# tlsfuzzer/tlslite-ng

Hardware: AMD Instinct MI355X
Metric: GiB/s device-resident record seal/open, AES-128-GCM + ChaCha20-Poly1305 16KiB (higher is better)
Workload: dtype u8

## Files before the change

tlslite-ng_amd/csrc/aes_bs.h:

```cpp
#pragma once
#include <stdint.h>
#if defined(__HIPCC__)
#include <hip/hip_runtime.h>
#endif

#if defined(__HIPCC__)
#define TG_BS_HD __host__ __device__ __forceinline__
#define TG_BS_MF __host__ __device__ __forceinline__
#else
#define TG_BS_HD static inline
#define TG_BS_MF inline
#endif

namespace tg {
namespace bs {

TG_BS_HD uint32_t bitmask(uint32_t w, int p) { return (uint32_t)((int32_t)(w << (31 - p)) >> 31); }

#if defined(__HIP_DEVICE_COMPILE__)
#define bop3(a, b, c, tt) __builtin_amdgcn_bitop3_b32((a), (b), (c), (tt))
#else
TG_BS_HD uint32_t bop3(uint32_t a, uint32_t b, uint32_t c, uint32_t tt) {
    uint32_t r = 0;
    for (int k = 0; k < 8; ++k)
        if ((tt >> k) & 1) r |= ((k & 4) ? a : ~a) & ((k & 2) ? b : ~b) & ((k & 1) ? c : ~c);
    return r;
}
#endif
TG_BS_HD uint32_t xor3(uint32_t a, uint32_t b, uint32_t c) { return bop3(a, b, c, 0x96); }

TG_BS_HD uint32_t perm(uint32_t hi, uint32_t lo, uint32_t sel) {
#if defined(__HIP_DEVICE_COMPILE__)
    return __builtin_amdgcn_perm(hi, lo, sel);
#else
    const uint64_t v = ((uint64_t)hi << 32) | lo;
    uint32_t r = 0;
    for (int i = 0; i < 4; ++i) r |= (uint32_t)((v >> (8 * ((sel >> (8 * i)) & 7))) & 0xff) << (8 * i);
    return r;
#endif
}

#include "aes_bs_sbox.h"

}
}
```

tlslite-ng_amd/csrc/aes_bs8.h:

```cpp
#pragma once
#include "aes_bs.h"
#include "keymath.h"

namespace tg {
namespace bs8 {

#if !defined(__HIP_DEVICE_COMPILE__)
using bs::bop3;
#endif
using bs::perm;
using bs::xor3;

TG_BS_HD uint32_t rotr_bytes(uint32_t x, int i) {
#if defined(__HIP_DEVICE_COMPILE__)
    return __builtin_amdgcn_alignbit(x, x, 8 * i);
#else
    return i ? (x >> (8 * i)) | (x << (32 - 8 * i)) : x;
#endif
}

TG_BS_HD uint32_t mask_word(const uint32_t* rk, int e) { return bs8_mask_word(rk, e); }

#if defined(__HIPCC__)
using Word4 = uint4;
// ... 206 lines not shown
            const uint32_t cw[4] = {c[b].x, c[b].y, c[b].z, c[b].w};
#pragma unroll
            for (int i = 0; i < 4; ++i) T[i] = xor3(a[i], a[(i + 1) & 3], cw[i]);
        }
#pragma unroll
        for (int i = 0; i < 4; ++i) {
            const uint32_t Tprev = b == 0 ? T7[i] : Tp[i];
            if (b == 1 || b == 3 || b == 4)
                s[i][b] = xor3(Tprev, T7[i], a[(i + 1) & 3]) ^ T[(i + 2) & 3];
            else
                s[i][b] = xor3(Tprev, a[(i + 1) & 3], T[(i + 2) & 3]);
        }
#pragma unroll
        for (int i = 0; i < 4; ++i) Tp[i] = T[i];
        TG_BS8_FENCE();
    }
}

struct TransposeMasks {
    uint32_t m4, m2, m1;
};
TG_BS_HD TransposeMasks transpose_masks() {
    TransposeMasks t{0x0f0f0f0fu, 0x33333333u, 0x55555555u};
#if defined(__HIP_DEVICE_COMPILE__)
    asm volatile("v_mov_b32 %0, 0x0f0f0f0f" : "=v"(t.m4));
    asm volatile("v_mov_b32 %0, 0x33333333" : "=v"(t.m2));
    asm volatile("v_mov_b32 %0, 0x55555555" : "=v"(t.m1));
#endif
    return t;
}

TG_BS_HD void transpose8(uint32_t* a, const TransposeMasks& tm) {
#pragma unroll
    for (int l = 2; l >= 0; --l) {
        const int m = 1 << l;
        const uint32_t mask = m == 4 ? tm.m4 : m == 2 ? tm.m2 : tm.m1;
#pragma unroll
        for (int r = 0; r < 8; ++r) {
            if (r & m) continue;
            const uint32_t x = a[r], y = a[r + m];
            uint32_t ys = y << m;
#if defined(__HIP_DEVICE_COMPILE__)
            if (m == 1) asm("v_add_u32 %0, %1, %1" : "=v"(ys) : "v"(y));
#endif
            a[r] = bop3(mask, x, ys, 0xca);
            a[r + m] = bop3(mask, x >> m, y, 0xca);
        }
    }
}

TG_BS_HD void to_blocks(uint32_t (*x)[8], uint32_t (*w)[8]) {
#pragma unroll
    for (int b = 0; b < 8; ++b) {
        const uint32_t s0 = x[0][b], s1 = x[1][b], s2 = x[2][b], s3 = x[3][b];
        const uint32_t A = perm(s1, s0, 0x07020500u);
        const uint32_t B = perm(s3, s2, 0x05000702u);
        const uint32_t A2 = perm(s1, s0, 0x04030601u);
        const uint32_t B2 = perm(s3, s2, 0x06010403u);
        w[0][b] = perm(B, A, 0x05040100u);
        w[2][b] = perm(B, A, 0x07060302u);
        w[1][b] = perm(B2, A2, 0x05040100u);
        w[3][b] = perm(B2, A2, 0x07060302u);
        TG_BS8_FENCE();
    }
    const TransposeMasks tm = transpose_masks();
#pragma unroll
    for (int q = 0; q < 4; ++q) {
        transpose8(w[q], tm);
        TG_BS8_FENCE();
    }
}

template <class KM, class = void>
struct RoundRows {
    static constexpr bool value = false;
};
template <class KM>
struct RoundRows<KM, decltype((void)KM::kRound)> {
    static constexpr bool value = KM::kRound;
};
template <class KM>
TG_BS_HD constexpr bool round_rows() { return RoundRows<KM>::value; }

template <int NR, class KM>
TG_BS_HD void encrypt(uint32_t (*s)[8], const KM& km, uint32_t (*w)[8], bool sub01 = true) {
    Word4 c[8];
    if constexpr (round_rows<KM>()) km.round(1, c);
    if (sub01) {
        bs::sbox(s[0]);
        TG_BS8_FENCE();
        bs::sbox(s[1]);
        TG_BS8_FENCE();
    }
    bs::sbox(s[2]);
    TG_BS8_FENCE();
    bs::sbox(s[3]);
    TG_BS8_FENCE();
    if constexpr (round_rows<KM>())
        mix_round_rows(s, c);
    else if constexpr (KM::kFolded)
        mix_round_folded(s, km, 1);
    else
        mix_round(s, km, 1);
#if defined(__HIP_DEVICE_COMPILE__)
#pragma unroll 1
#endif
    for (int r = 2; r < NR; ++r) {
        if constexpr (round_rows<KM>()) km.round(r, c);
#pragma unroll
        for (int i = 0; i < 4; ++i) {
            bs::sbox(s[i]);
            TG_BS8_FENCE();
        }
        if constexpr (round_rows<KM>())
            mix_round_rows(s, c);
        else if constexpr (KM::kFolded)
            mix_round_folded(s, km, r);
        else
            mix_round(s, km, r);
    }
#pragma unroll
    for (int i = 0; i < 4; ++i) {
        bs::sbox(s[i]);
        TG_BS8_FENCE();
    }
    to_blocks(s, w);
}

}
}
```

tlslite-ng_amd/csrc/aes_gcm_bs8.hip:

```cpp
#include <cstdlib>
#include <map>
#include <mutex>
#include <type_traits>
#include <utility>

#include "aes_bs8.h"
#include "aes_round.h"
#include "gcm_lane.h"
#include "ghash.h"
#include "options.h"
#include "runtime.h"

namespace tg {
namespace {

constexpr uint32_t kRecArea = 1536;

constexpr int kBs8Threads = 512;
constexpr int kBs8Recs = kBs8Threads / 8;
constexpr uint32_t kTeBase = 65536;
constexpr uint32_t kBs8Sbox = 65536;
constexpr uint32_t kBs8Jt = 65536 + 256;
constexpr uint32_t kBs8Keys = kBs8Jt + 256;
constexpr uint32_t kBs8RecBase = kBs8Keys + 2048;
constexpr size_t kBs8Lds = kBs8RecBase + (kBs8Threads / 64) * kRecArea;

extern __shared__ __attribute__((aligned(16))) uint4 g_lds_bs8[];

__device__ __forceinline__ uint32_t wave_max_u32(uint32_t v) {
#pragma unroll
    for (int off = 32; off >= 1; off >>= 1) {
        const uint32_t o = (uint32_t)__shfl_xor((int)v, off, 64);
        v = o > v ? o : v;
    }
    return __builtin_amdgcn_readfirstlane(v);
}

__device__ __forceinline__ uint32_t wave_min_u32(uint32_t v) {
#pragma unroll
    for (int off = 32; off >= 1; off >>= 1) {
        const uint32_t o = (uint32_t)__shfl_xor((int)v, off, 64);
        v = o < v ? o : v;
    }
    return __builtin_amdgcn_readfirstlane(v);
}

#if defined(TG_ROLE_PROBE)
__device__ unsigned long long g_rp[2][10];
struct RoleProbe {
    uint64_t last = 0;
    uint64_t acc[4] = {0, 0, 0, 0};
    __device__ __forceinline__ void start() { last = __builtin_amdgcn_s_memtime(); }
    __device__ __forceinline__ void mark(int k) {
        const uint64_t t = __builtin_amdgcn_s_memtime();
        acc[k] += t - last;
        last = t;
    }
    __device__ __forceinline__ void flush(bool trole, uint32_t blocks) {
        if ((threadIdx.x & 63u) == 0) {
            for (int k = 0; k < 4; ++k) atomicAdd(&g_rp[trole][k], (unsigned long long)acc[k]);
            atomicAdd(&g_rp[trole][5], 1ull);
            atomicAdd(&g_rp[trole][6], (unsigned long long)blocks);
        }
    }
};
__global__ void role_probe_print() {
    for (int r = 0; r < 2; ++r) {
        printf("ROLE_PROBE role %s setup %llu cipher %llu consume %llu tail %llu grab %llu jobs %llu blocks %llu span %llu waves %llu\n",
               r ? "ttable" : "bitsliced", g_rp[r][0], g_rp[r][1], g_rp[r][2], g_rp[r][3], g_rp[r][4], g_rp[r][5],
               g_rp[r][6], g_rp[r][7], g_rp[r][8]);
        for (int k = 0; k < 10; ++k) g_rp[r][k] = 0;
    }
}
#else
struct RoleProbe {
    __device__ __forceinline__ void start() {}
    __device__ __forceinline__ void mark(int) {}
    __device__ __forceinline__ void flush(bool, uint32_t) {}
};
#endif


template <int NR, int LPR = 8, class RK = RkLds>
__device__ __forceinline__ void t_half(uint32_t lane4, const RK& rk, const CtrCache& cc,
                                       uint32_t c0, bool win, const uint4& wc, uint32_t k0w, int h,
                                       uint4 (&ks)[4]) {
    uint32_t s[4][4];
#pragma unroll
    for (int q = 0; q < 4; ++q) {
        const uint32_t ctr = c0 + (uint32_t)LPR * (4 * h + q);
        if (win) {
            const uint32_t A = cc.k0 ^ rotl32(T2<3>((ctr << 24) ^ k0w, lane4), 8);
            s[q][0] = wc.x ^ T0<0>(A, lane4);
            s[q][1] = wc.y ^ rotl32(T2<3>(A, lane4), 8);
            s[q][2] = wc.z ^ T2<2>(A, lane4);
            s[q][3] = wc.w ^ rotl32(T0<1>(A, lane4), 8);
        } else {
            const uint32_t s3 = bswap32(ctr) ^ k0w;
            const uint32_t a0 = cc.k0 ^ rotl32(T2<3>(s3, lane4), 8);
            const uint32_t a1 = cc.k1 ^ T2<2>(s3, lane4);
            const uint32_t a2 = cc.k2 ^ rotl32(T0<1>(s3, lane4), 8);
            const uint32_t a3 = cc.k3 ^ T0<0>(s3, lane4);
            const uint4 k = rk.rot[2];
            s[q][0] = col_r(a0, a1, a2, a3, k.x, lane4);
            s[q][1] = col_r(a1, a2, a3, a0, k.y, lane4);
            s[q][2] = col_r(a2, a3, a0, a1, k.z, lane4);
            s[q][3] = col_r(a3, a0, a1, a2, k.w, lane4);
        }
    }
#if defined(TG_T_UNROLL)
#pragma unroll
#elif defined(TG_T_UNROLL1)
#pragma unroll 1
#else
#pragma unroll 2
#endif
    for (int r = 3; r < NR; ++r) {
        const uint4 k = rk.rot[r];
#pragma unroll
        for (int q = 0; q < 4; ++q) {
            const uint32_t t0 = col_r(s[q][0], s[q][1], s[q][2], s[q][3], k.x, lane4);
            const uint32_t t1 = col_r(s[q][1], s[q][2], s[q][3], s[q][0], k.y, lane4);
            const uint32_t t2 = col_r(s[q][2], s[q][3], s[q][0], s[q][1], k.z, lane4);
            const uint32_t t3 = col_r(s[q][3], s[q][0], s[q][1], s[q][2], k.w, lane4);
            s[q][0] = t0; s[q][1] = t1; s[q][2] = t2; s[q][3] = t3;
        }
    }
    const uint4 k = rk.rot[NR + 1];
#pragma unroll
    for (int q = 0; q < 4; ++q)
        ks[q] = make_uint4(col_last(s[q][0], s[q][1], s[q][2], s[q][3], k.x, lane4),
                           col_last(s[q][1], s[q][2], s[q][3], s[q][0], k.y, lane4),
                           col_last(s[q][2], s[q][3], s[q][0], s[q][1], k.z, lane4),
                           col_last(s[q][3], s[q][0], s[q][1], s[q][2], k.w, lane4));
}

struct SingleKeyCtx {
    const GcmKeyDev* key;
    uint32_t jt;
    __device__ __forceinline__ const uint32_t* rk() const { return key->rk; }
    __device__ __forceinline__ uint4 hpow(int e) const { return key->hpow[e - 1]; }
    __device__ __forceinline__ uint4 gmul(uint4 y) const { return gmul_rot(y, threadIdx.x & 15u, jt); }
    __device__ __forceinline__ uint4 gmulx(uint4 y, uint4 x) const { return gmul_rot(y, threadIdx.x & 15u, jt, x); }
    __device__ __forceinline__ const uint4* masks() const { return nullptr; }
};
struct SingleKeyRowCtx {
    const GcmKeyDev* key;
    uint4 jw;
    const uint4* mt = nullptr;
    uint32_t tid = threadIdx.x;
    __device__ __forceinline__ const uint32_t* rk() const { return key->rk; }
    __device__ __forceinline__ uint4 hpow(int e) const { return key->hpow[e - 1]; }
    __device__ __forceinline__ uint4 gmul(uint4 y) const { return gmul_rot_j(y, tid & 15u, jw); }
    __device__ __forceinline__ uint4 gmulx(uint4 y, uint4 x) const { return gmul_rot_j(y, tid & 15u, jw, x); }
    __device__ __forceinline__ const uint4* masks() const { return mt; }
};
struct TableKeyCtx {
    const uint32_t* rkw;
    const uint4* hp;
    uint32_t tab;
    const uint4* mt = nullptr;
    __device__ __forceinline__ const uint32_t* rk() const { return rkw; }
    __device__ __forceinline__ const uint4* masks() const { return mt; }
    __device__ __forceinline__ uint4 hpow(int e) const { return hp[e - 1]; }
#if defined(TG_KT_NO_GHASH)
    __device__ __forceinline__ uint4 gmul(uint4 y) const { return y; }
#else
    __device__ __forceinline__ uint4 gmul(uint4 y) const { return gmul4(y, tab); }
#endif
#if defined(TG_KT_NO_GHASH)
    __device__ __forceinline__ uint4 gmulx(uint4 y, uint4 x) const { return xor4(y, x); }
#else
    __device__ __forceinline__ uint4 gmulx(uint4 y, uint4 x) const { return gmul4(y, tab, x); }
#endif
};

template <int NR, bool OPEN, bool TROLE, class KM, class KC, bool PRE = false, int LPR = 8,
          class RKT = RkLds>
__device__ __forceinline__ void octet_job(const KC& kc, const tg_batch& b,
                                          const uint32_t* __restrict__ order, uint64_t t0,
                                          uint32_t recw, const RKT& rkT, uint32_t sbox,
                                          const KM& km, uint32_t tid = threadIdx.x) {
    static_assert(LPR == 8 || LPR == 16 || LPR == 32 || LPR == 64, "lanes per record");
    static_assert(LPR == 8 || LPR == 32 || !TROLE, "the T-table role runs octets or pairs");
    constexpr uint32_t kM = LPR - 1, kS = LPR == 8 ? 3 : LPR == 16 ? 4 : LPR == 32 ? 5 : 6;
    const uint32_t* rk = kc.rk();
    constexpr bool kNt = true;
    constexpr bool kShortT = !TROLE && LPR == 32 && std::is_same<RKT, RkTab>::value;
#if !defined(TG_KT_SHORT_MAX)
#define TG_KT_SHORT_MAX 5
#endif
    constexpr uint32_t kShortMax = TG_KT_SHORT_MAX;
    RoleProbe pr;
    if constexpr (LPR == 8) pr.start();
    const uint32_t lane = tid & 63u;
    const uint32_t l = lane & kM;
    const uint64_t t = t0 + (lane >> kS);
    const bool valid = t < b.n;
    const uint64_t i = valid ? (order ? gld(order, t) : t) : 0;
    uint32_t len = 0, alen = 0;
    const uint8_t* in = nullptr;
    uint8_t* out = nullptr;
    const uint8_t* ad = nullptr;
    uint4 nv = make_uint4(0, 0, 0, 0);
    if (valid) {
        len = rec_len(b, i);
        alen = rec_aad_len(b, i);
        in = rec_in(b, i);
        out = rec_out(b, i);
        ad = rec_aad(b, i);
        nv = load_partial(b.nonce + 12 * i, 12);
    }
    const uint32_t nfull = len >> 4, tail = len & 15, nc = (len + 15) >> 4, na = (alen + 15) >> 4;
    const uint32_t rho = (l + nc + 1u) & kM;
    const uint32_t recb = recw + (lane >> kS) * 128u;
    const uint32_t rsub = recw + (64u >> kS) * 128u + (lane >> kS) * 64u;
    const uint32_t lane4 = ((lane & 31u) << 2) | kTeBase;
    CtrCache cc = {0, 0, 0, 0};
    if (TROLE) {
        cc = ctr_cache<NR>(lane4, rkT, nv);
    } else {
        const uint32_t u[4] = {nv.x ^ rk[0], nv.y ^ rk[1], nv.z ^ rk[2], rk[3]};
        const uint32_t e = 4 * (l & 7u);
        const uint4 rp = make_uint4(bs8::rec_plane(u, e), bs8::rec_plane(u, e + 1),
                                    bs8::rec_plane(u, e + 2), bs8::rec_plane(u, e + 3));
        if (l < 8) lds_st128(recb + 16u * l, rp);
        __builtin_amdgcn_wave_barrier();
        uint32_t r[8];
        const uint4 a = lds_u128(recb + 32u * (l & 1u)), c = lds_u128(recb + 32u * (l & 1u) + 16u);
        r[0] = a.x; r[1] = a.y; r[2] = a.z; r[3] = a.w; r[4] = c.x; r[5] = c.y; r[6] = c.z; r[7] = c.w;
        bs::sbox(r);
        if (l < 2) {
            lds_st128(rsub + 32u * l, make_uint4(r[0], r[1], r[2], r[3]));
            lds_st128(rsub + 32u * l + 16u, make_uint4(r[4], r[5], r[6], r[7]));
        }
        __builtin_amdgcn_wave_barrier();
    }
    const bool aligned = (((uintptr_t)in | (uintptr_t)out) & 15) == 0;
    const uint32_t nvl = nc > rho ? (nc - rho + kM) >> kS : 0u;
    const uint32_t nfl = nfull > rho ? (nfull - rho + kM) >> kS : 0u;
    const uint32_t nbatch = wave_max_u32((nvl + 7u) >> 3);
    const uint32_t nfast = wave_min_u32(valid ? nfl >> 3 : 0xffffffffu);
    const uint4* mt = kc.masks();

    uint4 y = make_uint4(0, 0, 0, 0);
    for (uint32_t a = (l + na + nc + 1u) & kM; a < na; a += LPR) {
        const uint32_t m = alen - 16 * a < 16 ? alen - 16 * a : 16;
        y = kc.gmulx(y, load_partial(ad + 16 * a, m));
    }
    if constexpr (LPR == 8) pr.mark(0);

    uint4 rkl = make_uint4(0, 0, 0, 0);
    if constexpr (!TROLE) {
        if constexpr (bs8::round_rows<KM>()) {
            const uint4 v = gload16(reinterpret_cast<const uint8_t*>(rk + 4 * NR) + km.zv);
            rkl = make_uint4(v.x ^ 0x63636363u, v.y ^ 0x63636363u, v.z ^ 0x63636363u, v.w ^ 0x63636363u);
        } else {
            rkl = make_uint4(rk[4 * NR] ^ 0x63636363u, rk[4 * NR + 1] ^ 0x63636363u,
                             rk[4 * NR + 2] ^ 0x63636363u, rk[4 * NR + 3] ^ 0x63636363u);
        }
    }
    auto consume = [&](const uint4* ks, uint32_t blk0, int j0, auto NN, const uint4* pre) {
        constexpr int N = decltype(NN)::value;
        if (blk0 < (nfast << (kS + 3))) {
            if (valid) {
                uint4 d[N];
#pragma unroll
                for (int q = 0; q < N; ++q)
                    d[q] = pre ? pre[q]
                               : kNt ? gload16u_nt(in + 16u * (blk0 + LPR * (j0 + q)))
                                     : gload16u(in + 16u * (blk0 + LPR * (j0 + q)));
#pragma unroll
                for (int q = 0; q < N; ++q) {
                    const uint4 k = ks[q];
                    const uint4 c = make_uint4(xor3(d[q].x, k.x, rkl.x), xor3(d[q].y, k.y, rkl.y),
                                               xor3(d[q].z, k.z, rkl.z), xor3(d[q].w, k.w, rkl.w));
                    if constexpr (kNt)
                        gstore16u_nt(out + 16u * (blk0 + LPR * (j0 + q)), c);
                    else
                        gstore16u(out + 16u * (blk0 + LPR * (j0 + q)), c);
                    if (!OPEN) d[q] = c;
                }
#pragma unroll
                for (int q = 0; q < N; ++q) y = kc.gmulx(y, d[q]);
            }
        } else {
#pragma unroll
            for (int q = 0; q < N; ++q) {
                const uint32_t blk = blk0 + LPR * (j0 + q);
                if (!valid || blk >= nc) continue;
                const uint4 k = ks[q];
                const uint4 kk = make_uint4(k.x ^ rkl.x, k.y ^ rkl.y, k.z ^ rkl.z, k.w ^ rkl.w);
                uint4 d, c;
                if (blk < nfull) {
                    d = load16(in + 16u * blk, aligned);
                    c = xor4(d, kk);
                    store16(out + 16u * blk, c, aligned);
                } else {
                    d = load_partial(in + 16u * blk, tail);
                    c = mask_tail(xor4(d, kk), tail);
                    store_partial(out + 16u * blk, c, tail);
                }
                y = kc.gmulx(y, OPEN ? d : c);
            }
        }
    };
    for (uint32_t beta = 0; beta < nbatch; ++beta) {
        const uint32_t blk0 = rho + 8u * LPR * beta;
        const uint32_t c0 = 2u + blk0;
        const bool one = !OPEN && __all(!valid || nvl <= 8u * beta + 1u);
        if (!OPEN && mt && __all(!valid || nvl <= 8u * beta || (nvl == 8u * beta + 1u && blk0 == nc - 1u))) {
            uint4 ks[1] = {rkl};
            if (valid && nvl == 8u * beta + 1u) {
#if defined(TG_DEBUG_ASSERT)
                assert(lone_last_block<LPR>(nc));
#endif
                ks[0] = xor4(gload16(reinterpret_cast<const uint8_t*>(mt + 2 * t + 1)), rkl);
            }
            consume(ks, blk0, 0, std::integral_constant<int, 1>(), nullptr);
        } else if (TROLE) {
            const bool win = __all(((c0 ^ (c0 + 7u * LPR)) >> 8) == 0);
            const uint32_t k0w = rkT.get(0).w;
            const uint4 wc = LPR == 8 && win ? win_consts<NR>(lane4, rkT, cc, c0) : make_uint4(0, 0, 0, 0);
#if defined(TG_T_UNROLL)
#pragma unroll
#else
#pragma unroll 1
#endif
            for (int h = 0; h < 2; ++h) {
                if (h == 1 && __all(!valid || nvl <= 8u * beta + 4u)) break;
                uint4 ks[4];
                uint4 dp[4];
                const bool fast = blk0 < (nfast << (kS + 3));
                if (fast && valid) {
#pragma unroll
                    for (int q = 0; q < 4; ++q)
                        dp[q] = kNt ? gload16u_nt(in + 16u * (blk0 + LPR * (4 * h + q)))
                                    : gload16u(in + 16u * (blk0 + LPR * (4 * h + q)));
                }
                if constexpr (LPR == 8) {
                    t_half<NR>(lane4, rkT, cc, c0, win, wc, k0w, h, ks);
                } else {
                    const uint32_t ch = c0 + 4u * LPR * h;
                    const bool winh = __all(((ch ^ (ch + 3u * LPR)) >> 8) == 0);
                    const uint4 wch = winh ? win_consts<NR>(lane4, rkT, cc, ch) : make_uint4(0, 0, 0, 0);
                    t_half<NR, LPR>(lane4, rkT, cc, c0, winh, wch, k0w, h, ks);
                }
                if constexpr (LPR == 8) pr.mark(1);
                consume(ks, blk0, 4 * h, std::integral_constant<int, 4>(), fast ? dp : nullptr);
                if constexpr (LPR == 8) pr.mark(2);
                __builtin_amdgcn_sched_barrier(0);
            }
        } else if (!OPEN && one) {
            const uint4 nvr = valid ? load_partial(b.nonce + 12 * i, 12) : make_uint4(0, 0, 0, 0);
            uint4 ks[1] = {xor4(aes_block_sb<NR>(rk, make_uint4(nvr.x, nvr.y, nvr.z, bswap32(c0)), sbox), rkl)};
            consume(ks, blk0, 0, std::integral_constant<int, 1>(), nullptr);
        } else if (kShortT && __all(!valid || nvl < 8u * beta + kShortMax)) {
            const CtrCache cct = ctr_cache<NR>(lane4, rkT, nv);
#pragma unroll 1
            for (int h = 0; h < 2; ++h) {
                if (h == 1 && __all(!valid || nvl <= 8u * beta + 4u)) break;
                const uint32_t ch = c0 + 4u * LPR * h;
                const bool winh = __all(((ch ^ (ch + 3u * LPR)) >> 8) == 0);
                const uint4 wch = winh ? win_consts<NR>(lane4, rkT, cct, ch) : make_uint4(0, 0, 0, 0);
                uint4 ks[4];
                t_half<NR, LPR>(lane4, rkT, cct, c0, winh, wch, rkT.get(0).w, h, ks);
#pragma unroll
                for (int q = 0; q < 4; ++q) ks[q] = xor4(ks[q], rkl);
                consume(ks, blk0, 4 * h, std::integral_constant<int, 4>(), nullptr);
            }
        } else {
            const bool hi = (beta + 1u) >> (16 - (kS + 3));
            uint32_t s[4][8];
#pragma unroll
            for (int q = 0; q < 8; ++q) {
                const uint4 v = lds_u128((q < 4 && !hi ? rsub : recb) + 16u * q);
                s[q >> 1][4 * (q & 1) + 0] = v.x;
                s[q >> 1][4 * (q & 1) + 1] = v.y;
                s[q >> 1][4 * (q & 1) + 2] = v.z;
                s[q >> 1][4 * (q & 1) + 3] = v.w;
            }
            uint32_t lanec[kS + 3], kmask;
            bs8::lane_consts<kS>(c0, lanec, kmask);
#pragma unroll
            for (int bb = 0; bb < (int)kS + 3; ++bb) s[3 - (bb >> 3)][bb & 7] ^= lanec[bb];
            bs8::ctr_planes<kS + 3, 16, kS + 3>(s, kmask, beta);
            if (hi) bs8::ctr_planes<16, 32, kS + 3>(s, kmask, beta);
            uint4 dp[8];
            const bool pre = PRE && blk0 < (nfast << (kS + 3));
            if (pre && valid) {
#pragma unroll
                for (int q = 0; q < 8; ++q)
                    dp[q] = kNt ? gload16u_nt(in + 16u * (blk0 + LPR * q)) : gload16u(in + 16u * (blk0 + LPR * q));
            }

            uint32_t w[4][8];
            bs8::encrypt<NR>(s, km, w, hi);
            uint4 ks[8];
#pragma unroll
            for (int j = 0; j < 8; ++j) ks[j] = make_uint4(w[0][j], w[1][j], w[2][j], w[3][j]);
            if constexpr (LPR == 8) pr.mark(1);
            consume(ks, blk0, 0, std::integral_constant<int, 8>(), pre ? dp : nullptr);
            if constexpr (LPR == 8) pr.mark(2);
        }
    }
    if constexpr (LPR == 8) pr.mark(2);
#if defined(TG_ROLE_PROBE)
    uint32_t pblk = (valid && l == 0) ? nc : 0u;
    for (int m = 8; m < 64; m <<= 1) pblk += (uint32_t)__shfl_xor((int)pblk, m, 64);
#endif
    if (!__any(valid)) {
#if defined(TG_ROLE_PROBE)
        if constexpr (LPR == 8) pr.flush(TROLE, pblk);
#endif
        return;
    }
    if (l == kM) {
        const uint64_t abits = (uint64_t)alen << 3, cbits = (uint64_t)len << 3;
        y = kc.gmulx(y, make_uint4(bswap32((uint32_t)(abits >> 32)), bswap32((uint32_t)abits),
                                     bswap32((uint32_t)(cbits >> 32)), bswap32((uint32_t)cbits)));
    }
    uint4 mask = make_uint4(0, 0, 0, 0);
    if (mt && valid) mask = gload16(reinterpret_cast<const uint8_t*>(mt + 2 * t));
    uint4 yn = norm4(y);
    if (yn.x | yn.y | yn.z | yn.w) yn = gf128_mul(yn, kc.hpow(LPR - l));
#pragma unroll
    for (int m = 1; m < LPR; m <<= 1) yn = xor4(yn, shfl_xor4(yn, m));
    if (!mt) {
        if (valid) nv = load_partial(b.nonce + 12 * i, 12);
        mask = TROLE ? aes_ctr<NR>(lane4, rkT, cc, 1u)
                     : aes_block_sb<NR>(rk, make_uint4(nv.x, nv.y, nv.z, bswap32(1u)), sbox);
    }
    const uint4 tag = xor4(norm4(yn), mask);
    const bool tag_aligned = aligned && tail == 0;
    if (!OPEN) {
        if (valid && l == 0) store16(out + len, tag, tag_aligned);
#if defined(TG_ROLE_PROBE)
        if constexpr (LPR == 8) {
            pr.mark(3);
            pr.flush(TROLE, pblk);
        }
#endif
        return;
    }
    uint32_t diff = 0;
    if (valid && l == 0) {
        const uint4 exp = load16(in + len, tag_aligned);
        diff = (exp.x ^ tag.x) | (exp.y ^ tag.y) | (exp.z ^ tag.z) | (exp.w ^ tag.w);
        if (b.status) gst(b.status, i, (uint8_t)(diff == 0));
    }
    diff = (uint32_t)__shfl((int)diff, (int)(lane & ~kM & 63u), 64);
    if (valid && diff) {
        const uint32_t rz = ((fresh_lane() & kM) + nc + 1u) & kM;
        const uint4 z = make_uint4(0, 0, 0, 0);
        for (uint32_t blk = rz; blk < nfull; blk += LPR) store16(out + 16u * blk, z, aligned);
        if (tail && (nfull & kM) == rz) store_partial(out + 16u * nfull, z, tail);
    }
#if defined(TG_ROLE_PROBE)
    if constexpr (LPR == 8) {
        pr.mark(3);
        pr.flush(TROLE, pblk);
    }
#endif
}

__device__ __forceinline__ void stage_sbox(uint32_t base) {
    if (threadIdx.x < 64) {
        uint32_t v = 0;
#pragma unroll
        for (int q = 0; q < 4; ++q) v |= ((c_te.te0[4 * threadIdx.x + q] >> 8) & 0xffu) << (8 * q);
        reinterpret_cast<uint32_t*>(g_lds_bs8)[base / 4 + threadIdx.x] = v;
    }
}

template <int NR, bool OPEN>
__global__ __launch_bounds__(kBs8Threads, 4) void gcm_bs8_kernel(const GcmKeyDev* __restrict__ key,
                                                                tg_batch b,
                                                                const uint32_t* __restrict__ order) {
    stage_ghash_rot(g_lds_bs8, key->ghash8, kBs8Jt);
    stage_sbox(kBs8Sbox);
    bs8::stage_lds_planes(kBs8Keys, key->bs8mask, NR);
    __syncthreads();
    const uint32_t wave = threadIdx.x >> 6;
    octet_job<NR, OPEN, false>(SingleKeyCtx{key, kBs8Jt}, b, order,
                               (uint64_t)blockIdx.x * kBs8Recs + 8u * wave,
                               kBs8RecBase + wave * kRecArea, RkLds{0}, kBs8Sbox,
                               bs8::KeyPlanesLds{kBs8Keys});
}

constexpr int kHyThreads = 1024;
constexpr uint32_t kHySbox = 2 * 65536;
constexpr uint32_t kHyRk = kHySbox + 256;
constexpr uint32_t kHyJt = kHyRk + 256;
constexpr uint32_t kHyKeys = kHyJt + 256;
constexpr uint32_t kHyRecBase = kHyKeys + 2048;
constexpr size_t kHyLds = kHyRecBase + (kHyThreads / 64) * kRecArea;
static_assert(kTeBase == 65536, "Te block follows the GHASH tables");

#if defined(TG_TAIL_PROBE)
__device__ unsigned long long g_tp[8] = {~0ull, 0, ~0ull, 0, 0, 0, 0, 0};
__device__ __forceinline__ void tail_probe_start() {
    if ((threadIdx.x & 63u) == 0) atomicMin(&g_tp[0], (unsigned long long)__builtin_amdgcn_s_memrealtime());
}
__device__ __forceinline__ void tail_probe_end(bool trole) {
    if ((threadIdx.x & 63u) == 0) {
        const unsigned long long t = __builtin_amdgcn_s_memrealtime();
        atomicMax(&g_tp[1], t);
        atomicMin(&g_tp[2], t);
        atomicAdd(&g_tp[3], t - g_tp[0]);
        atomicAdd(&g_tp[4], 1ull);
        atomicMax(&g_tp[trole ? 5 : 6], t);
    }
}
__global__ void tail_probe_print() {
    const unsigned long long t0 = g_tp[0];
    printf("TAIL_PROBE kernel_us %.1f first_end_us %.1f mean_end_us %.1f last_T_us %.1f last_bs_us %.1f waves %llu\n",
           (g_tp[1] - t0) / 100.0, (g_tp[2] - t0) / 100.0, g_tp[3] / (100.0 * g_tp[4]), (g_tp[5] - t0) / 100.0,
           (g_tp[6] - t0) / 100.0, g_tp[4]);
    g_tp[0] = ~0ull; g_tp[1] = 0; g_tp[2] = ~0ull; g_tp[3] = 0; g_tp[4] = 0; g_tp[5] = 0; g_tp[6] = 0;
}
#endif

#if defined(TG_HY_HOIST)
__device__ __forceinline__ uint32_t hy_tid(uint32_t) { return threadIdx.x; }
#else
__device__ __forceinline__ uint32_t hy_tid(uint32_t wave) { return (wave << 6) | fresh_lane(); }
#endif
template <int NR, bool OPEN, int THREADS>
__global__ __launch_bounds__(THREADS) void gcm_hy_kernel(const GcmKeyDev* __restrict__ key,
                                                            const tg_batch* __restrict__ bp,
                                                            const uint32_t* __restrict__ order,
                                                            uint32_t* __restrict__ queue,
                                                            uint32_t nt, uint32_t prio,
                                                            const uint4* __restrict__ krows,
                                                            const uint4* __restrict__ rkrot,
                                                            const uint4* __restrict__ masks) {
    stage_ghash_rot(g_lds_bs8, key->ghash8, kHyJt);
    stage_te(reinterpret_cast<uint32_t*>(g_lds_bs8) + kTeBase / 4);
    stage_sbox(kHySbox);
    if (threadIdx.x < 4 * (NR + 1)) reinterpret_cast<uint32_t*>(g_lds_bs8)[kHyRk / 4 + threadIdx.x] = key->rk[threadIdx.x];
    __syncthreads();
    const uint32_t wave = (uint32_t)__builtin_amdgcn_readfirstlane((int)(threadIdx.x >> 6));
#if defined(TG_TAIL_PROBE)
    tail_probe_start();
#endif
    const uint64_t njobs = (bp->n + 7) / 8;
    const uint32_t recw = kHyRecBase + wave * kRecArea;
#if defined(TG_ROLE_PROBE)
    const uint64_t rp_t0 = __builtin_amdgcn_s_memtime();
    uint64_t rp_grab = 0;
#define RP_GRAB_START const uint64_t rp_g0 = __builtin_amdgcn_s_memtime();
#define RP_GRAB_END rp_grab += __builtin_amdgcn_s_memtime() - rp_g0;
#else
#define RP_GRAB_START
#define RP_GRAB_END
#endif
    if (wave < nt) {
        if (prio) __builtin_amdgcn_s_setprio(1);
        const RkLds rk{kHyRk, rkrot};
        for (;;) {
            RP_GRAB_START
            uint32_t job = 0;
            if ((threadIdx.x & 63u) == 0) job = atomicAdd(queue, 1u);
            job = (uint32_t)__builtin_amdgcn_readfirstlane((int)job);
            RP_GRAB_END
            if (job >= njobs) break;
            asm volatile("" ::: "memory");
            const tg_batch b = *bp;
            const uint32_t tid = hy_tid(wave);
            const uint4 jw = lds_u128(kHyJt + ((tid & 15u) << 4));
            octet_job<NR, OPEN, true>(SingleKeyRowCtx{key, jw, masks, tid}, b, order, 8ull * job, recw, rk,
                                      kHySbox, bs8::KeyPlanesVmemFolded{{krows}}, tid);
        }
    } else {
        const RkLds none{0};
        for (;;) {
            RP_GRAB_START
            uint32_t job = 0;
            if ((threadIdx.x & 63u) == 0) job = atomicAdd(queue, 1u);
            job = (uint32_t)__builtin_amdgcn_readfirstlane((int)job);
            RP_GRAB_END
            if (job >= njobs) break;
            asm volatile("" ::: "memory");
            const tg_batch b = *bp;
            const uint32_t tid = hy_tid(wave);
            const uint4 jw = lds_u128(kHyJt + ((tid & 15u) << 4));
            octet_job<NR, OPEN, false, bs8::KeyPlanesVmemFolded, SingleKeyRowCtx, (THREADS < 1024)>(
                SingleKeyRowCtx{key, jw, masks, tid}, b, order, 8ull * job, recw, none, kHySbox,
                bs8::KeyPlanesVmemFolded{{krows}}, tid);
        }
    }
#if defined(TG_TAIL_PROBE)
    tail_probe_end(wave < nt);
#endif
#if defined(TG_ROLE_PROBE)
    if ((threadIdx.x & 63u) == 0) {
        const bool tr = wave < nt;
        atomicAdd(&g_rp[tr][4], (unsigned long long)rp_grab);
        atomicAdd(&g_rp[tr][7], (unsigned long long)(__builtin_amdgcn_s_memtime() - rp_t0));
        atomicAdd(&g_rp[tr][8], 1ull);
    }
#endif
#undef RP_GRAB_START
#undef RP_GRAB_END
}

__global__ void hy_setup_kernel(tg_batch b, uint32_t* queue, tg_batch* bcopy) {
    if (threadIdx.x == 0) {
        *queue = 0;
        *bcopy = b;
    }
}

template <int NR>
__global__ __launch_bounds__(1024) void hy_mask_kernel(const GcmKeyDev* __restrict__ key, tg_batch b,
                                                       const uint32_t* __restrict__ order,
                                                       uint4* __restrict__ masks) {
    stage_te(reinterpret_cast<uint32_t*>(g_lds_bs8));
    RkRegs<NR> rk;
#pragma unroll
    for (int k = 0; k < 4 * (NR + 1); ++k) rk.w[k] = key->rk[k];
    __syncthreads();
    const uint32_t lane4 = (threadIdx.x & 31u) << 2;
    for (uint64_t t = (uint64_t)blockIdx.x * blockDim.x + threadIdx.x; t < b.n;
         t += (uint64_t)gridDim.x * blockDim.x) {
        const uint64_t i = order ? gld(order, t) : t;
        const uint4 nv = load_partial(b.nonce + 12 * i, 12);
        gstore16(reinterpret_cast<uint8_t*>(masks + 2 * t),
                 aes_block<NR>(lane4, rk, make_uint4(nv.x, nv.y, nv.z, bswap32(1u))));
        const uint32_t nc = (rec_len(b, i) + 15) >> 4;
        if (lone_last_block<8>(nc))
            gstore16(reinterpret_cast<uint8_t*>(masks + 2 * t + 1),
                     aes_block<NR>(lane4, rk, make_uint4(nv.x, nv.y, nv.z, bswap32(nc + 1u))));
    }
}

template <int NR, bool OPEN>
int launch_bs8(const GcmKeyDev* key, const tg_batch& b, hipStream_t s, const uint32_t* order) {
    if (lds_attr((const void*)gcm_bs8_kernel<NR, OPEN>, (int)kBs8Lds)) return TG_EHIP;
    const uint64_t groups = (b.n + kBs8Recs - 1) / kBs8Recs;
    if (groups > 0x7fffffffull) return TG_EINVAL;
    hipLaunchKernelGGL((gcm_bs8_kernel<NR, OPEN>), dim3((unsigned)groups), dim3(kBs8Threads), kBs8Lds, s,
                       key, b, order);
    return hipGetLastError() == hipSuccess ? TG_OK : TG_EHIP;
}

template <int NR, bool OPEN>
int launch_hy_kernels(const GcmKeyDev* key, const tg_batch& b, hipStream_t s, const uint32_t* order, uint32_t nt,
                      uint32_t prio, bool small, uint32_t* queue, tg_batch* bcopy, uint4* masks) {
    if (masks && b.n) {
        if (lds_attr((const void*)hy_mask_kernel<NR>, 65536)) return TG_EHIP;
        const uint64_t wgs = (b.n + 1023) / 1024, cus = (uint64_t)device_cus();
        const unsigned grid = (unsigned)(wgs < cus ? wgs : cus);
        hipLaunchKernelGGL((hy_mask_kernel<NR>), dim3(grid), dim3(1024), 65536, s, key, b, order, masks);
        if (hipGetLastError() != hipSuccess) return TG_EHIP;
    }
    const uint4* krows = reinterpret_cast<const uint4*>(key->bs8rows);
    const uint4* rkrot = reinterpret_cast<const uint4*>(key->rkrot);
    if (small)
        hipLaunchKernelGGL((gcm_hy_kernel<NR, OPEN, 768>), dim3((unsigned)device_cus()), dim3(768), kHyLds, s,
                           key, (const tg_batch*)bcopy, order, queue, nt, prio, krows, rkrot, masks);
    else
        hipLaunchKernelGGL((gcm_hy_kernel<NR, OPEN, 1024>), dim3((unsigned)device_cus()), dim3(1024), kHyLds,
                           s, key, (const tg_batch*)bcopy, order, queue, nt, prio, krows, rkrot, masks);
#if defined(TG_TAIL_PROBE)
    hipLaunchKernelGGL(tail_probe_print, dim3(1), dim3(1), 0, s);
#endif
#if defined(TG_ROLE_PROBE)
    hipLaunchKernelGGL(role_probe_print, dim3(1), dim3(1), 0, s);
#endif
    return hipGetLastError() == hipSuccess ? TG_OK : TG_EHIP;
}
// ... 377 lines not shown
```

Measured before the change: 1489.

## Cache per-window first-two-round AES state in LDS for hybrid GCM kernel

Adds a windowed counter path to the hybrid GCM kernel. For each 256-counter window, the first two AES rounds of the fixed nonce/high-counter bytes are precomputed once and kept in per-wave LDS areas, along with a key-dependent table covering the varying low counter byte. Bitsliced waves then start at round 3 instead of recomputing rounds 1-2, and T-table waves read the window constants from LDS instead of recomputing them per call. LDS layout is reorganised, with optional double buffering across window boundaries, which adds scalar setup work, extra LDS traffic and wave barriers in exchange for fewer full AES rounds per block.

```diff
diff --git a/tlslite-ng_amd/csrc/aes_bs.h b/tlslite-ng_amd/csrc/aes_bs.h
--- a/tlslite-ng_amd/csrc/aes_bs.h
+++ b/tlslite-ng_amd/csrc/aes_bs.h
@@ -35,7 +35,10 @@
 #else
     const uint64_t v = ((uint64_t)hi << 32) | lo;
     uint32_t r = 0;
-    for (int i = 0; i < 4; ++i) r |= (uint32_t)((v >> (8 * ((sel >> (8 * i)) & 7))) & 0xff) << (8 * i);
+    for (int i = 0; i < 4; ++i) {
+        const uint32_t k = (sel >> (8 * i)) & 0xff;
+        if (k < 8) r |= (uint32_t)((v >> (8 * k)) & 0xff) << (8 * i);
+    }
     return r;
 #endif
 }
diff --git a/tlslite-ng_amd/csrc/aes_bs8.h b/tlslite-ng_amd/csrc/aes_bs8.h
--- a/tlslite-ng_amd/csrc/aes_bs8.h
+++ b/tlslite-ng_amd/csrc/aes_bs8.h
@@ -312,8 +312,8 @@
 template <class KM>
 TG_BS_HD constexpr bool round_rows() { return RoundRows<KM>::value; }
 
-template <int NR, class KM>
-TG_BS_HD void encrypt(uint32_t (*s)[8], const KM& km, uint32_t (*w)[8], bool sub01 = true) {
+template <class KM>
+TG_BS_HD void round1(uint32_t (*s)[8], const KM& km, bool sub01 = true) {
     Word4 c[8];
     if constexpr (round_rows<KM>()) km.round(1, c);
     if (sub01) {
@@ -332,10 +332,15 @@
         mix_round_folded(s, km, 1);
     else
         mix_round(s, km, 1);
+}
+
+template <int NR, class KM>
+TG_BS_HD void rounds_from(uint32_t (*s)[8], const KM& km, uint32_t (*w)[8], int r0) {
+    Word4 c[8];
 #if defined(__HIP_DEVICE_COMPILE__)
 #pragma unroll 1
 #endif
-    for (int r = 2; r < NR; ++r) {
+    for (int r = r0; r < NR; ++r) {
         if constexpr (round_rows<KM>()) km.round(r, c);
 #pragma unroll
         for (int i = 0; i < 4; ++i) {
@@ -357,5 +362,100 @@
     to_blocks(s, w);
 }
 
-}
-}
+template <int NR, class KM>
+TG_BS_HD void encrypt(uint32_t (*s)[8], const KM& km, uint32_t (*w)[8], bool sub01 = true) {
+    round1(s, km, sub01);
+    rounds_from<NR>(s, km, w, 2);
+}
+
+
+template <class SB>
+TG_BS_HD uint32_t sub4(uint32_t w, const SB& sb) {
+    return sb(w & 0xffu) | (sb((w >> 8) & 0xffu) << 8) | (sb((w >> 16) & 0xffu) << 16) | (sb(w >> 24) << 24);
+}
+
+TG_BS_HD uint32_t mix_col(uint32_t w) {
+    const uint32_t r1 = rotr_bytes(w, 1), r2 = rotr_bytes(w, 2), r3 = rotr_bytes(w, 3);
+    const uint32_t u = w ^ r1;
+    const uint32_t xt = ((u & 0x7f7f7f7fu) << 1) ^ (((u >> 7) & 0x01010101u) * 0x1bu);
+    return xt ^ xor3(r1, r2, r3);
+}
+
+TG_BS_HD uint32_t shift_col(const uint32_t s[4], int c) {
+    return (s[c] & 0x000000ffu) | (s[(c + 1) & 3] & 0x0000ff00u) | (s[(c + 2) & 3] & 0x00ff0000u) |
+           (s[(c + 3) & 3] & 0xff000000u);
+}
+
+template <class SB>
+TG_BS_HD void win_words(const uint32_t* rk, uint32_t n0, uint32_t n1, uint32_t n2, uint32_t win, const SB& sb,
+                        uint32_t& A, uint32_t (&B)[4]) {
+    const uint32_t cw = ((win >> 16) & 0xffu) | (win & 0xff00u) | ((win & 0xffu) << 16);
+    const uint32_t s[4] = {n0 ^ rk[0], n1 ^ rk[1], n2 ^ rk[2], cw ^ rk[3]};
+    uint32_t a[4];
+    A = mix_col(sub4(shift_col(s, 0), sb) & 0x00ffffffu) ^ rk[4];
+    a[0] = 0;
+#if defined(__HIP_DEVICE_COMPILE__)
+#pragma unroll
+#endif
+    for (int c = 1; c < 4; ++c) a[c] = mix_col(sub4(shift_col(s, c), sb)) ^ rk[4 + c];
+#if defined(__HIP_DEVICE_COMPILE__)
+#pragma unroll
+#endif
+    for (int c = 0; c < 4; ++c) B[c] = mix_col(sub4(shift_col(a, c), sb)) ^ rk[8 + c];
+}
+
+TG_BS_HD uint32_t a_plane(uint32_t A, uint32_t b) { return ((A >> b) & 0x01010101u) * 0xffu; }
+
+template <class SB>
+TG_BS_HD uint32_t v_word(uint32_t k15, uint32_t rho, uint32_t bm, uint32_t b, const SB& sb) {
+    uint32_t w = 0;
+    for (uint32_t j = 0; j < 8; ++j) {
+        const uint32_t s = sb(((2u + rho + 8u * j + 64u * bm) & 0xffu) ^ k15);
+        const uint32_t s2 = ((s << 1) ^ ((s & 0x80u) ? 0x11bu : 0u)) & 0xffu;
+        const uint32_t col = s | (s << 8) | ((s2 ^ s) << 16) | (s2 << 24);
+        w |= ((col >> b) & 0x01010101u) << j;
+    }
+    return w;
+}
+
+TG_BS_HD void first_state(const uint32_t u[4], uint32_t c0, uint32_t beta, bool hi, uint32_t (*s)[8]) {
+#if defined(__HIP_DEVICE_COMPILE__)
+#pragma unroll
+#endif
+    for (int e = 0; e < 32; ++e) s[e >> 3][e & 7] = rec_plane(u, e);
+    uint32_t lanec[6], kmask;
+    lane_consts<3>(c0, lanec, kmask);
+#if defined(__HIP_DEVICE_COMPILE__)
+#pragma unroll
+#endif
+    for (int b = 0; b < 6; ++b) s[3][b] ^= lanec[b];
+    ctr_planes<6, 16, 6>(s, kmask, beta);
+    if (hi) ctr_planes<16, 32, 6>(s, kmask, beta);
+}
+
+TG_BS_HD uint32_t win_m7(uint32_t kmask) { return kmask & 0x80808080u; }
+TG_BS_HD uint32_t win_sel7(uint32_t cur, uint32_t next, uint32_t m7) { return bop3(m7, next, cur, 0xca); }
+
+template <class BP>
+TG_BS_HD void win_rounds(uint32_t (&x)[8], const BP& bp, uint32_t (*s)[8]) {
+    bs::sbox(x);
+    TG_BS8_FENCE();
+#if defined(__HIP_DEVICE_COMPILE__)
+#pragma unroll
+#endif
+    for (int b = 0; b < 8; ++b) {
+        const uint32_t p = x[(b + 7) & 7];
+        const uint32_t y2 = b == 0 ? p : (b == 1 || b == 3 || b == 4) ? p ^ x[7] : p;
+        const uint32_t y3 = b == 0 ? p ^ x[0] : (b == 1 || b == 3 || b == 4) ? xor3(p, x[7], x[b]) : p ^ x[b];
+        const uint32_t z = perm(x[b], x[b], 0x01020300u);
+        const Word4 k = bp(b);
+        s[0][b] = xor3(z, perm(y3, y2, 0x010c0c04u), k.x);
+        s[1][b] = xor3(z, perm(y3, y2, 0x05020c0cu), k.y);
+        s[2][b] = xor3(z, perm(y3, y2, 0x0c06030cu), k.z);
+        s[3][b] = xor3(z, perm(y3, y2, 0x0c0c0700u), k.w);
+        TG_BS8_FENCE();
+    }
+}
+
+}
+}
diff --git a/tlslite-ng_amd/csrc/aes_gcm_bs8.hip b/tlslite-ng_amd/csrc/aes_gcm_bs8.hip
--- a/tlslite-ng_amd/csrc/aes_gcm_bs8.hip
+++ b/tlslite-ng_amd/csrc/aes_gcm_bs8.hip
@@ -26,6 +26,34 @@
 constexpr size_t kBs8Lds = kBs8RecBase + (kBs8Threads / 64) * kRecArea;
 
 extern __shared__ __attribute__((aligned(16))) uint4 g_lds_bs8[];
+
+struct SboxLds {
+    uint32_t base;
+    __device__ __forceinline__ uint32_t operator()(uint32_t x) const { return lds_u8(base + x); }
+};
+struct WinPlanes {
+    uint32_t cur, nxt, m7;
+    bool cross;
+    __device__ __forceinline__ uint4 operator()(int b) const {
+        uint4 v = lds_u128(cur + 128u * b);
+        if (cross) {
+            const uint4 n = lds_u128(nxt + 128u * b);
+            v = make_uint4(bs8::win_sel7(v.x, n.x, m7), bs8::win_sel7(v.y, n.y, m7), bs8::win_sel7(v.z, n.z, m7),
+                           bs8::win_sel7(v.w, n.w, m7));
+        }
+        return v;
+    }
+};
+struct SboxTe {
+    __device__ __forceinline__ uint32_t operator()(uint32_t x) const { return (c_te.te0[x] >> 8) & 0xffu; }
+};
+
+__device__ __forceinline__ void stage_vtab(uint32_t base, uint32_t k15) {
+    const uint32_t e = threadIdx.x;
+    if (e < 256)
+        reinterpret_cast<uint32_t*>(g_lds_bs8)[base / 4 + e] =
+            bs8::v_word(k15, (e >> 2) & 7u, e >> 6, 4u * ((e >> 5) & 1u) + (e & 3u), SboxTe());
+}
 
 __device__ __forceinline__ uint32_t wave_max_u32(uint32_t v) {
 #pragma unroll
@@ -81,20 +109,22 @@
 #endif
 
 
-template <int NR, int LPR = 8, class RK = RkLds>
+template <int NR, int LPR = 8, class RK = RkLds, bool WLDS = false>
 __device__ __forceinline__ void t_half(uint32_t lane4, const RK& rk, const CtrCache& cc,
-                                       uint32_t c0, bool win, const uint4& wc, uint32_t k0w, int h,
-                                       uint4 (&ks)[4]) {
+                                       uint32_t c0, bool win, const uint4& wc0, uint32_t k0w, int h,
+                                       uint4 (&ks)[4], uint32_t wcur = 0, uint32_t w7 = 0) {
     uint32_t s[4][4];
+    const uint4 wc = WLDS ? lds_u128(wcur) : wc0;
 #pragma unroll
     for (int q = 0; q < 4; ++q) {
         const uint32_t ctr = c0 + (uint32_t)LPR * (4 * h + q);
-        if (win) {
+        if (WLDS || win) {
+            const uint4 wq = WLDS && q == 3 ? lds_u128(h ? w7 : wcur) : wc;
             const uint32_t A = cc.k0 ^ rotl32(T2<3>((ctr << 24) ^ k0w, lane4), 8);
-            s[q][0] = wc.x ^ T0<0>(A, lane4);
-            s[q][1] = wc.y ^ rotl32(T2<3>(A, lane4), 8);
-            s[q][2] = wc.z ^ T2<2>(A, lane4);
-            s[q][3] = wc.w ^ rotl32(T0<1>(A, lane4), 8);
+            s[q][0] = wq.x ^ T0<0>(A, lane4);
+            s[q][1] = wq.y ^ rotl32(T2<3>(A, lane4), 8);
+            s[q][2] = wq.z ^ T2<2>(A, lane4);
+            s[q][3] = wq.w ^ rotl32(T0<1>(A, lane4), 8);
         } else {
             const uint32_t s3 = bswap32(ctr) ^ k0w;
             const uint32_t a0 = cc.k0 ^ rotl32(T2<3>(s3, lane4), 8);
@@ -176,13 +206,15 @@
 };
 
 template <int NR, bool OPEN, bool TROLE, class KM, class KC, bool PRE = false, int LPR = 8,
-          class RKT = RkLds>
+          class RKT = RkLds, bool WIN = false>
 __device__ __forceinline__ void octet_job(const KC& kc, const tg_batch& b,
                                           const uint32_t* __restrict__ order, uint64_t t0,
                                           uint32_t recw, const RKT& rkT, uint32_t sbox,
-                                          const KM& km, uint32_t tid = threadIdx.x) {
+                                          const KM& km, uint32_t tid = threadIdx.x, uint32_t vtab = 0,
+                                          bool dbl = false) {
     static_assert(LPR == 8 || LPR == 16 || LPR == 32 || LPR == 64, "lanes per record");
     static_assert(LPR == 8 || LPR == 32 || !TROLE, "the T-table role runs octets or pairs");
+    static_assert(!WIN || LPR == 8, "the window areas: octets");
     constexpr uint32_t kM = LPR - 1, kS = LPR == 8 ? 3 : LPR == 16 ? 4 : LPR == 32 ? 5 : 6;
     const uint32_t* rk = kc.rk();
     constexpr bool kNt = true;
@@ -219,7 +251,7 @@
     CtrCache cc = {0, 0, 0, 0};
     if (TROLE) {
         cc = ctr_cache<NR>(lane4, rkT, nv);
-    } else {
+    } else if constexpr (!WIN) {
         const uint32_t u[4] = {nv.x ^ rk[0], nv.y ^ rk[1], nv.z ^ rk[2], rk[3]};
         const uint32_t e = 4 * (l & 7u);
         const uint4 rp = make_uint4(bs8::rec_plane(u, e), bs8::rec_plane(u, e + 1),
@@ -242,6 +274,7 @@
     const uint32_t nbatch = wave_max_u32((nvl + 7u) >> 3);
     const uint32_t nfast = wave_min_u32(valid ? nfl >> 3 : 0xffffffffu);
     const uint4* mt = kc.masks();
+    auto slot = [&]() { return t0 + ((fresh_lane() & 63u) >> kS); };
 
     uint4 y = make_uint4(0, 0, 0, 0);
     for (uint32_t a = (l + na + nc + 1u) & kM; a < na; a += LPR) {
@@ -315,13 +348,24 @@
 #if defined(TG_DEBUG_ASSERT)
                 assert(lone_last_block<LPR>(nc));
 #endif
-                ks[0] = xor4(gload16(reinterpret_cast<const uint8_t*>(mt + 2 * t + 1)), rkl);
+                ks[0] = xor4(gload16(reinterpret_cast<const uint8_t*>(mt + 2 * slot() + 1)), rkl);
             }
             consume(ks, blk0, 0, std::integral_constant<int, 1>(), nullptr);
         } else if (TROLE) {
-            const bool win = __all(((c0 ^ (c0 + 7u * LPR)) >> 8) == 0);
+            constexpr bool kTWin = WIN && LPR == 8;
+            const bool win = kTWin || __all(((c0 ^ (c0 + 7u * LPR)) >> 8) == 0);
             const uint32_t k0w = rkT.get(0).w;
-            const uint4 wc = LPR == 8 && win ? win_consts<NR>(lane4, rkT, cc, c0) : make_uint4(0, 0, 0, 0);
+            const uint4 wc = LPR == 8 && win && !kTWin ? win_consts<NR>(lane4, rkT, cc, c0) : make_uint4(0, 0, 0, 0);
+            uint32_t wcur = 0, w7 = 0;
+            if constexpr (kTWin) {
+                const uint32_t wsl = recw + 16u * (lane >> 3), wnd = beta >> 2;
+                const bool cross = (beta & 3u) == 3u;
+                if (beta == 0) lds_st128(wsl, win_consts<NR>(lane4, rkT, cc, 0u));
+                if (cross) lds_st128(wsl + 128u * ((wnd + 1u) & 1u), win_consts<NR>(lane4, rkT, cc, (wnd + 1u) << 8));
+                __builtin_amdgcn_wave_barrier();
+                wcur = wsl + 128u * (wnd & 1u);
+                w7 = cross && ((c0 >> 3) & 1u) ? wsl + 128u * ((wnd + 1u) & 1u) : wcur;
+            }
 #if defined(TG_T_UNROLL)
 #pragma unroll
 #else
@@ -339,7 +383,7 @@
                                     : gload16u(in + 16u * (blk0 + LPR * (4 * h + q)));
                 }
                 if constexpr (LPR == 8) {
-                    t_half<NR>(lane4, rkT, cc, c0, win, wc, k0w, h, ks);
+                    t_half<NR, 8, RKT, kTWin>(lane4, rkT, cc, c0, win, wc, k0w, h, ks, wcur, w7);
                 } else {
                     const uint32_t ch = c0 + 4u * LPR * h;
                     const bool winh = __all(((ch ^ (ch + 3u * LPR)) >> 8) == 0);
@@ -372,20 +416,54 @@
         } else {
             const bool hi = (beta + 1u) >> (16 - (kS + 3));
             uint32_t s[4][8];
-#pragma unroll
-            for (int q = 0; q < 8; ++q) {
-                const uint4 v = lds_u128((q < 4 && !hi ? rsub : recb) + 16u * q);
-                s[q >> 1][4 * (q & 1) + 0] = v.x;
-                s[q >> 1][4 * (q & 1) + 1] = v.y;
-                s[q >> 1][4 * (q & 1) + 2] = v.z;
-                s[q >> 1][4 * (q & 1) + 3] = v.w;
-            }
-            uint32_t lanec[kS + 3], kmask;
-            bs8::lane_consts<kS>(c0, lanec, kmask);
-#pragma unroll
-            for (int bb = 0; bb < (int)kS + 3; ++bb) s[3 - (bb >> 3)][bb & 7] ^= lanec[bb];
-            bs8::ctr_planes<kS + 3, 16, kS + 3>(s, kmask, beta);
-            if (hi) bs8::ctr_planes<16, 32, kS + 3>(s, kmask, beta);
+            bool win = false;
+            if constexpr (WIN) {
+                const uint32_t q16 = 16u * (lane >> 3);
+                const uint32_t bbase = recw + 256u + q16, wnd = beta >> 2;
+                const bool cross = (beta & 3u) == 3u;
+                win = !hi && (dbl || !cross);
+                const bool first = (beta & 3u) == 0 && (beta == 0 || !dbl);
+                if (!hi && (first || (cross && dbl))) {
+                    const uint32_t wn = first ? wnd : wnd + 1u;
+                    const uint4 nvr = load_partial(b.nonce + 12 * i, 12);
+                    uint32_t A, Bw[4];
+                    bs8::win_words(rk, nvr.x, nvr.y, nvr.z, wn, SboxLds{sbox}, A, Bw);
+                    lds_st128(bbase + (dbl ? 1024u * (wn & 1u) : 0u) + 128u * l,
+                              make_uint4(bs8::rec_plane(Bw, l), bs8::rec_plane(Bw, 8 + l),
+                                         bs8::rec_plane(Bw, 16 + l), bs8::rec_plane(Bw, 24 + l)));
+                    lds_st32(recw + q16 + 128u * (l >> 2) + 4u * (l & 3u), bs8::a_plane(A, l));
+                    __builtin_amdgcn_wave_barrier();
+                }
+                if (win) {
+                    const uint32_t va = vtab + 256u * (beta & 3u) + 16u * (rho & 7u);
+                    const uint4 a0 = lds_u128(recw + q16), a1 = lds_u128(recw + q16 + 128u);
+                    const uint4 v0 = lds_u128(va), v1 = lds_u128(va + 128u);
+                    uint32_t x[8] = {a0.x ^ v0.x, a0.y ^ v0.y, a0.z ^ v0.z, a0.w ^ v0.w,
+                                     a1.x ^ v1.x, a1.y ^ v1.y, a1.z ^ v1.z, a1.w ^ v1.w};
+                    bs8::win_rounds(x, WinPlanes{bbase + (dbl ? 1024u * (wnd & 1u) : 0u),
+                                                 bbase + 1024u * ((wnd + 1u) & 1u),
+                                                 bs8::win_m7((c0 >> 3) & 1u ? 0xffffffffu : 0u), cross}, s);
+                } else {
+                    const uint4 nvr = load_partial(b.nonce + 12 * i, 12);
+                    const uint32_t u[4] = {nvr.x ^ rk[0], nvr.y ^ rk[1], nvr.z ^ rk[2], rk[3]};
+                    bs8::first_state(u, c0, beta, hi, s);
+                }
+            } else {
+#pragma unroll
+                for (int q = 0; q < 8; ++q) {
+                    const uint4 v = lds_u128((q < 4 && !hi ? rsub : recb) + 16u * q);
+                    s[q >> 1][4 * (q & 1) + 0] = v.x;
+                    s[q >> 1][4 * (q & 1) + 1] = v.y;
+                    s[q >> 1][4 * (q & 1) + 2] = v.z;
+                    s[q >> 1][4 * (q & 1) + 3] = v.w;
+                }
+                uint32_t lanec[kS + 3], kmask;
+                bs8::lane_consts<kS>(c0, lanec, kmask);
+#pragma unroll
+                for (int bb = 0; bb < (int)kS + 3; ++bb) s[3 - (bb >> 3)][bb & 7] ^= lanec[bb];
+                bs8::ctr_planes<kS + 3, 16, kS + 3>(s, kmask, beta);
+                if (hi) bs8::ctr_planes<16, 32, kS + 3>(s, kmask, beta);
+            }
             uint4 dp[8];
             const bool pre = PRE && blk0 < (nfast << (kS + 3));
             if (pre && valid) {
@@ -395,7 +473,8 @@
             }
 
             uint32_t w[4][8];
-            bs8::encrypt<NR>(s, km, w, hi);
+            if (!win) bs8::round1(s, km, WIN || hi);
+            bs8::rounds_from<NR>(s, km, w, win ? 3 : 2);
             uint4 ks[8];
 #pragma unroll
             for (int j = 0; j < 8; ++j) ks[j] = make_uint4(w[0][j], w[1][j], w[2][j], w[3][j]);
@@ -421,7 +500,7 @@
                                      bswap32((uint32_t)(cbits >> 32)), bswap32((uint32_t)cbits)));
     }
     uint4 mask = make_uint4(0, 0, 0, 0);
-    if (mt && valid) mask = gload16(reinterpret_cast<const uint8_t*>(mt + 2 * t));
+    if (mt && valid) mask = gload16(reinterpret_cast<const uint8_t*>(mt + 2 * slot()));
     uint4 yn = norm4(y);
     if (yn.x | yn.y | yn.z | yn.w) yn = gf128_mul(yn, kc.hpow(LPR - l));
 #pragma unroll
@@ -452,7 +531,9 @@
     diff = (uint32_t)__shfl((int)diff, (int)(lane & ~kM & 63u), 64);
     if (valid && diff) {
         const uint32_t rz = ((fresh_lane() & kM) + nc + 1u) & kM;
-        const uint4 z = make_uint4(0, 0, 0, 0);
+        uint32_t z0 = 0;
+        asm volatile("" : "+v"(z0));
+        const uint4 z = make_uint4(z0, z0, z0, z0);
         for (uint32_t blk = rz; blk < nfull; blk += LPR) store16(out + 16u * blk, z, aligned);
         if (tail && (nfull & kM) == rz) store_partial(out + 16u * nfull, z, tail);
     }
@@ -492,9 +573,18 @@
 constexpr uint32_t kHySbox = 2 * 65536;
 constexpr uint32_t kHyRk = kHySbox + 256;
 constexpr uint32_t kHyJt = kHyRk + 256;
-constexpr uint32_t kHyKeys = kHyJt + 256;
-constexpr uint32_t kHyRecBase = kHyKeys + 2048;
-constexpr size_t kHyLds = kHyRecBase + (kHyThreads / 64) * kRecArea;
+constexpr uint32_t kHyV = kHyJt + 256;
+constexpr uint32_t kHyWin = kHyV + 1024;
+constexpr uint32_t kHyBsArea = 256 + 2 * 1024, kHyBsArea1 = 256 + 1024;
+constexpr uint32_t kHyTArea = 2 * 128;
+constexpr size_t kHyLds = kHyWin + 13 * kHyBsArea;
+static_assert(kHyLds <= 163840 && kHyWin + (kHyThreads / 64) * kHyBsArea1 <= kHyLds, "hybrid LDS");
+#if defined(TG_HY_NO_WIN)
+constexpr bool kHyWinPath = false;
+static_assert(kHyWin + (kHyThreads / 64) * kRecArea <= kHyLds, "hybrid LDS");
+#else
+constexpr bool kHyWinPath = true;
+#endif
 static_assert(kTeBase == 65536, "Te block follows the GHASH tables");
 
 #if defined(TG_TAIL_PROBE)
@@ -539,13 +629,18 @@
     stage_te(reinterpret_cast<uint32_t*>(g_lds_bs8) + kTeBase / 4);
     stage_sbox(kHySbox);
     if (threadIdx.x < 4 * (NR + 1)) reinterpret_cast<uint32_t*>(g_lds_bs8)[kHyRk / 4 + threadIdx.x] = key->rk[threadIdx.x];
+    if constexpr (kHyWinPath) stage_vtab(kHyV, key->rk[3] >> 24);
     __syncthreads();
     const uint32_t wave = (uint32_t)__builtin_amdgcn_readfirstlane((int)(threadIdx.x >> 6));
 #if defined(TG_TAIL_PROBE)
     tail_probe_start();
 #endif
     const uint64_t njobs = (bp->n + 7) / 8;
-    const uint32_t recw = kHyRecBase + wave * kRecArea;
+    const bool dbl = nt * kHyTArea + (THREADS / 64 - nt) * kHyBsArea <= kHyLds - kHyWin;
+    const uint32_t recw = (uint32_t)__builtin_amdgcn_readfirstlane(
+        (int)(!kHyWinPath ? kHyWin + wave * kRecArea
+              : wave < nt ? kHyWin + wave * kHyTArea
+                          : kHyWin + nt * kHyTArea + (wave - nt) * (dbl ? kHyBsArea : kHyBsArea1)));
 #if defined(TG_ROLE_PROBE)
     const uint64_t rp_t0 = __builtin_amdgcn_s_memtime();
     uint64_t rp_grab = 0;
@@ -561,7 +656,7 @@
         for (;;) {
             RP_GRAB_START
             uint32_t job = 0;
-            if ((threadIdx.x & 63u) == 0) job = atomicAdd(queue, 1u);
+            if (fresh_lane() == 0) job = atomicAdd(queue, 1u);
             job = (uint32_t)__builtin_amdgcn_readfirstlane((int)job);
             RP_GRAB_END
             if (job >= njobs) break;
@@ -569,15 +664,16 @@
             const tg_batch b = *bp;
             const uint32_t tid = hy_tid(wave);
             const uint4 jw = lds_u128(kHyJt + ((tid & 15u) << 4));
-            octet_job<NR, OPEN, true>(SingleKeyRowCtx{key, jw, masks, tid}, b, order, 8ull * job, recw, rk,
-                                      kHySbox, bs8::KeyPlanesVmemFolded{{krows}}, tid);
+            octet_job<NR, OPEN, true, bs8::KeyPlanesVmemFolded, SingleKeyRowCtx, false, 8, RkLds, kHyWinPath>(
+                SingleKeyRowCtx{key, jw, masks, tid}, b, order, 8ull * job, recw, rk, kHySbox,
+                bs8::KeyPlanesVmemFolded{{krows}}, tid);
         }
     } else {
         const RkLds none{0};
         for (;;) {
             RP_GRAB_START
             uint32_t job = 0;
-            if ((threadIdx.x & 63u) == 0) job = atomicAdd(queue, 1u);
+            if (fresh_lane() == 0) job = atomicAdd(queue, 1u);
             job = (uint32_t)__builtin_amdgcn_readfirstlane((int)job);
             RP_GRAB_END
             if (job >= njobs) break;
@@ -585,9 +681,9 @@
             const tg_batch b = *bp;
             const uint32_t tid = hy_tid(wave);
             const uint4 jw = lds_u128(kHyJt + ((tid & 15u) << 4));
-            octet_job<NR, OPEN, false, bs8::KeyPlanesVmemFolded, SingleKeyRowCtx, (THREADS < 1024)>(
-                SingleKeyRowCtx{key, jw, masks, tid}, b, order, 8ull * job, recw, none, kHySbox,
-                bs8::KeyPlanesVmemFolded{{krows}}, tid);
+            octet_job<NR, OPEN, false, bs8::KeyPlanesVmemFolded, SingleKeyRowCtx, (THREADS < 1024), 8, RkLds,
+                      kHyWinPath>(SingleKeyRowCtx{key, jw, masks, tid}, b, order, 8ull * job, recw, none, kHySbox,
+                                  bs8::KeyPlanesVmemFolded{{krows}}, tid, kHyV, dbl);
         }
     }
 #if defined(TG_TAIL_PROBE)
```

Result: faster. 1513, median of 6 (+1.6%).
